# tictacmenthe/F2CNN

Hardware: AMD Instinct MI355X
Metric: audio-seconds/sec through filterbank+envelope (HIP, 1 MI355X per rank); the +CNN figure of BASELINE's metric is value_with_cnn / blocks.cfg4 (higher is better)
Workload: dtype f64 filter state + f64 utterance FFT + f32 row FFT; 1 GPU; cfg3: filterbank + Hilbert envelope + 50 Hz LPF in one call (f32 FFT), batch of 1000 x 1 s utterances per GPU, 128 channels, ENV1 (float64) out; channels=128, lpf_hz=50, launch_batch=1000, outputs_resident_in_hbm=True, parallelism=utterance-sharded x1, no collective, utterances_sent_back_by_the_accuracy_guard=0

## Files before the change

f2cnn_amd/csrc/f2_spectral.hip:

```cpp
#define f2fft f2fft_sp
#undef F2_PLAN13_PASSES
#define F2_PLAN13_PASSES 4
#include <algorithm>
#include <cmath>
#include <complex>
#include <thread>

#include "f2_fft_lds.h"

using namespace f2fft;

namespace {

typedef float f2_f4 __attribute__((ext_vector_type(4)));
constexpr int SPEC_GB = 16;

constexpr int KS_CGROUP = 32;
constexpr int KS_CGROUP_LONG = 8;
constexpr int KS_STORE_AUX = 2;
typedef unsigned int f2_u4 __attribute__((ext_vector_type(4)));
typedef unsigned int f2_u2 __attribute__((ext_vector_type(2)));
__device__ __forceinline__ __amdgpu_buffer_rsrc_t row_buffer(double* y, int n) {
    return __builtin_amdgcn_make_buffer_rsrc(y, 0, n * 8, 0x00020000);
}
__device__ __forceinline__ __amdgpu_buffer_rsrc_t row_buffer_uniform(double* y, int n) {
    const unsigned long long a = (unsigned long long)y;
    const unsigned lo = __builtin_amdgcn_readfirstlane((unsigned)a), hi = __builtin_amdgcn_readfirstlane((unsigned)(a >> 32));
    return row_buffer((double*)(((unsigned long long)hi << 32) | lo), __builtin_amdgcn_readfirstlane(n));
}
__device__ __forceinline__ void store_row_pair_inside(__amdgpu_buffer_rsrc_t r, int i0, double a, double b) {
    const f2_d2 v = {a, b};
    __builtin_amdgcn_raw_buffer_store_b128(__builtin_bit_cast(f2_u4, v), r, i0 * 8, 0, KS_STORE_AUX);
}
__device__ __forceinline__ void store_row_pair_buf(__amdgpu_buffer_rsrc_t r, int n, int i0, double a, double b) {
    if (i0 + 1 < n) {
        const f2_d2 v = {a, b};
        __builtin_amdgcn_raw_buffer_store_b128(__builtin_bit_cast(f2_u4, v), r, i0 * 8, 0, KS_STORE_AUX);
    } else if (i0 < n) {
        __builtin_amdgcn_raw_buffer_store_b64(__builtin_bit_cast(f2_u2, a), r, i0 * 8, 0, KS_STORE_AUX);
    }
}

struct LowpassConsts {
    float qf, b0f;
    float g1, g2, g4, g8;
    double gw, gblk;
};

template <int NT, int NBLK>
constexpr size_t lowpass_tab_lds_bytes() {
    return sizeof(float) * (2 * (size_t)NBLK * (NT / 64) + NBLK);
}

#define F2_DPP_STEP(CTRL)                                                                                                    \
    asm volatile("s_nop 1\n\t"                                                                                               \
                 "v_fmac_f32_dpp %0, %0, %16 " CTRL "\n\t"                                                                   \
                 "v_fmac_f32_dpp %1, %1, %16 " CTRL "\n\t"                                                                   \
                 "v_fmac_f32_dpp %2, %2, %16 " CTRL "\n\t"                                                                   \
                 "v_fmac_f32_dpp %3, %3, %16 " CTRL "\n\t"                                                                   \
                 "v_fmac_f32_dpp %4, %4, %16 " CTRL "\n\t"                                                                   \
                 "v_fmac_f32_dpp %5, %5, %16 " CTRL "\n\t"                                                                   \
                 "v_fmac_f32_dpp %6, %6, %16 " CTRL "\n\t"                                                                   \
                 "v_fmac_f32_dpp %7, %7, %16 " CTRL "\n\t"                                                                   \
                 "v_fmac_f32_dpp %8, %8, %16 " CTRL "\n\t"                                                                   \
                 "v_fmac_f32_dpp %9, %9, %16 " CTRL "\n\t"                                                                   \
                 "v_fmac_f32_dpp %10, %10, %16 " CTRL "\n\t"                                                                 \
                 "v_fmac_f32_dpp %11, %11, %16 " CTRL "\n\t"                                                                 \
                 "v_fmac_f32_dpp %12, %12, %16 " CTRL "\n\t"                                                                 \
                 "v_fmac_f32_dpp %13, %13, %16 " CTRL "\n\t"                                                                 \
                 "v_fmac_f32_dpp %14, %14, %16 " CTRL "\n\t"                                                                 \
                 "v_fmac_f32_dpp %15, %15, %16 " CTRL                                                                        \
                 : "+v"(sc[0]), "+v"(sc[1]), "+v"(sc[2]), "+v"(sc[3]), "+v"(sc[4]), "+v"(sc[5]), "+v"(sc[6]), "+v"(sc[7]),   \
                   "+v"(sc[8]), "+v"(sc[9]), "+v"(sc[10]), "+v"(sc[11]), "+v"(sc[12]), "+v"(sc[13]), "+v"(sc[14]), "+v"(sc[15]) \
                 : "v"(mult))

template <int NT, int NBLK, bool CHAINED = false, bool INSIDE15 = false>
__device__ __forceinline__ float lowpass_pairs_store_tab(const float (&er)[NBLK], const float (&ei)[NBLK], const LowpassConsts& K,
                                                        const f2_f4* __restrict__ lptab, unsigned char* smem,
                                                        double* __restrict__ y, int n, int tid, int ibase = 0,
                                                        double* ychain = nullptr) {
    static_assert(NBLK == 16, "sixteen blocks: one DPP row chains them");
    constexpr int NW = NT / 64;
    float* wtot = reinterpret_cast<float*>(smem);
    float* cwl = wtot + NBLK * NW;
    float* ycar = cwl + NBLK * NW;
    const int lane = tid & 63, wv = tid >> 6;
    const f2_f4 tc = lptab[tid];
    float sc[NBLK];
#pragma unroll
    for (int jj = 0; jj < NBLK; ++jj) sc[jj] = fmaf(K.qf, er[jj], ei[jj]);
    {
        float mult = K.g1;
        F2_DPP_STEP("row_shr:1 row_mask:0xf bank_mask:0xf bound_ctrl:0");
        mult = K.g2;
        F2_DPP_STEP("row_shr:2 row_mask:0xf bank_mask:0xf bound_ctrl:0");
        mult = K.g4;
        F2_DPP_STEP("row_shr:4 row_mask:0xf bank_mask:0xf bound_ctrl:0");
        mult = K.g8;
        F2_DPP_STEP("row_shr:8 row_mask:0xf bank_mask:0xf bound_ctrl:0");
        mult = tc.z;
        F2_DPP_STEP("row_bcast:15 row_mask:0xa bank_mask:0xf");
        mult = tc.w;
        F2_DPP_STEP("row_bcast:31 row_mask:0xc bank_mask:0xf");
    }
    if (lane == 63) {
#pragma unroll
        for (int jj = 0; jj < NBLK; ++jj) wtot[jj * NW + wv] = sc[jj];
    }
    __syncthreads();
    if (tid < NBLK) {
        double c = 0.0;
#pragma unroll
        for (int w2 = 0; w2 < NW; ++w2) {
            cwl[tid * NW + w2] = (float)c;
            c = fma(K.gw, c, (double)wtot[tid * NW + w2]);
        }
        const double G1 = K.gblk, G2 = G1 * G1, G4 = G2 * G2, G8 = G4 * G4;
        double yin = 0.0;
        if constexpr (CHAINED) {
            yin = *ychain;
            if (tid == 0) c = fma(G1, yin, c);
        }
        c = fma(G1, dpp_mov<0x111, 0xF>(c), c);
        c = fma(G2, dpp_mov<0x112, 0xF>(c), c);
        c = fma(G4, dpp_mov<0x114, 0xF>(c), c);
        c = fma(G8, dpp_mov<0x118, 0xF>(c), c);
        const double cprev = dpp_mov<0x111, 0xF>(c);
        if constexpr (CHAINED) {
            ycar[tid] = tid == 0 ? (float)yin : (float)cprev;
            if (tid == NBLK - 1) *ychain = c;
        } else {
            ycar[tid] = (float)cprev;
        }
    }
    __syncthreads();
    const __amdgpu_buffer_rsrc_t yb = CHAINED ? row_buffer_uniform(y, n) : row_buffer(y, n);
    float ymax = 0.f;
#pragma unroll
    for (int jj = 0; jj < NBLK; ++jj) {
        const float cw = cwl[jj * NW + wv];
        const float sin_ = fmaf(tc.x, cw, sc[jj]);
        const float up = dpp_mov<0x138, 0xF>(sin_);
        const float sprev = lane > 0 ? up : cw;
        const float sp = fmaf(tc.y, ycar[jj], sprev);
        const float s0 = fmaf(K.qf, sp, er[jj]);
        const float s1 = fmaf(K.qf, s0, ei[jj]);
        const float y0 = K.b0f * (s0 + sp);
        const float y1 = K.b0f * (s1 + s0);
        const int i0 = ibase + 2 * (tid + NT * jj);
        if constexpr (INSIDE15) {
            if (jj < NBLK - 1) {
                store_row_pair_inside(yb, i0, (double)y0, (double)y1);
                ymax = fmaxf(ymax, fabsf(y1));
            } else {
                store_row_pair_buf(yb, n, i0, (double)y0, (double)y1);
                ymax = fmaxf(ymax, i0 + 1 < n ? fabsf(y1) : (i0 < n ? fabsf(y0) : 0.f));
            }
        } else if constexpr (CHAINED) {
            store_row_pair_buf(yb, n, i0, (double)y0, (double)y1);
            const int lo = ibase + 2 * NT * jj;
            if (lo + 2 * NT <= n) ymax = fmaxf(ymax, fabsf(y1));
            else if (lo < n) ymax = fmaxf(ymax, i0 + 1 < n ? fabsf(y1) : fabsf(y0));
        } else {
            const int lo = ibase + 2 * NT * jj;
            if (lo + 2 * NT <= n) {
                store_row_pair_inside(yb, i0, (double)y0, (double)y1);
                ymax = fmaxf(ymax, fabsf(y1));
            } else if (lo < n) {
                store_row_pair_buf(yb, n, i0, (double)y0, (double)y1);
                ymax = fmaxf(ymax, i0 + 1 < n ? fabsf(y1) : (i0 < n ? fabsf(y0) : 0.f));
            }
        }
    }
    return ymax;
}

struct SpecParams {
    int64_t xpitch;
    int64_t tpitch;
    double* env;
    int* uflag;
    int C;
    int nutt;
    int lpf;
    LowpassConsts lp;
    float tol;
    float* gdump;
    unsigned long long* stamps;
};

__device__ __forceinline__ cpx<float> spectral_bin(cpx<float> X, f2_f4 hu, cpx<float> w, cpx<float> z, const float* __restrict__ rho) {
    const float ur = hu.z, ui = hu.w;
    float tr = fmaf(rho[1], w.re, rho[0]), ti = rho[1] * w.im;
#pragma unroll
    for (int j = 1; j < 4; ++j) {
        const float rr = fmaf(rho[2 * j + 1], w.re, rho[2 * j]), ri = rho[2 * j + 1] * w.im;
        const float nr = fmaf(-ui, ti, fmaf(ur, tr, rr));
        const float ni = fmaf(ui, tr, fmaf(ur, ti, ri));
        tr = nr;
        ti = ni;
    }
    const float qr = ur * tr - ui * ti, qi = ur * ti + ui * tr;
    float yr = hu.x * X.re;
    yr = fmaf(-hu.y, X.im, yr);
    yr = fmaf(z.re, qr, yr);
    yr = fmaf(-z.im, qi, yr);
    float yi = hu.x * X.im;
    yi = fmaf(hu.y, X.re, yi);
    yi = fmaf(z.re, qi, yi);
    yi = fmaf(z.im, qr, yi);
    return {yr, yi};
}

#include "f2_fft13_merged.h"

template <int R0, int J = 0>
__device__ __forceinline__ cpx<float> bin_w(cpx<float> w0, int j) {
    if constexpr (J < R0) {
        if (j == J) return mulw<2 * R0, J>(w0);
        return bin_w<R0, J + 1>(w0, j);
    } else {
        return w0;
    }
}

#define F2_DPP_MAX2(CTRL)                                              \
    asm volatile("s_nop 1\n\t"                                         \
                 "v_max_f32_dpp %0, %0, %0 " CTRL "\n\t"               \
                 "v_max_f32_dpp %1, %1, %1 " CTRL                       \
                 : "+v"(a), "+v"(b))
__device__ __forceinline__ void wave_max63x2(float& a, float& b) {
    F2_DPP_MAX2("row_shr:1 row_mask:0xf bank_mask:0xf bound_ctrl:0");
    F2_DPP_MAX2("row_shr:2 row_mask:0xf bank_mask:0xf bound_ctrl:0");
    F2_DPP_MAX2("row_shr:4 row_mask:0xf bank_mask:0xf bound_ctrl:0");
    F2_DPP_MAX2("row_shr:8 row_mask:0xf bank_mask:0xf bound_ctrl:0");
    F2_DPP_MAX2("row_bcast:15 row_mask:0xa bank_mask:0xf");
    F2_DPP_MAX2("row_bcast:31 row_mask:0xc bank_mask:0xf");
}
__device__ __forceinline__ float wave_max63(float v) {
    asm volatile("s_nop 1\n\t"
                 "v_max_f32_dpp %0, %0, %0 row_shr:1 row_mask:0xf bank_mask:0xf bound_ctrl:0\n\ts_nop 1\n\t"
                 "v_max_f32_dpp %0, %0, %0 row_shr:2 row_mask:0xf bank_mask:0xf bound_ctrl:0\n\ts_nop 1\n\t"
                 "v_max_f32_dpp %0, %0, %0 row_shr:4 row_mask:0xf bank_mask:0xf bound_ctrl:0\n\ts_nop 1\n\t"
                 "v_max_f32_dpp %0, %0, %0 row_shr:8 row_mask:0xf bank_mask:0xf bound_ctrl:0\n\ts_nop 1\n\t"
                 "v_max_f32_dpp %0, %0, %0 row_bcast:15 row_mask:0xa bank_mask:0xf\n\ts_nop 1\n\t"
                 "v_max_f32_dpp %0, %0, %0 row_bcast:31 row_mask:0xc bank_mask:0xf"
                 : "+v"(v));
    return v;
}

template <int R0, int NT, bool PADLAST>
__device__ __forceinline__ float pad_residual(const cpx<float> (&v)[R0], int n, int tid, int odd, float gout) {
    if constexpr (PADLAST) {
        return fmaxf(gout, 2 * (tid + NT * (R0 - 1)) + odd >= n ? fabsf(v[brev<R0>(R0 - 1)].re) : 0.f);
    } else {
        int jmin = (n - 2 * tid - odd + 2 * NT - 1) >> (__builtin_ctz(2 * NT));
        asm volatile("" : "+v"(jmin));
#pragma unroll
        for (int j = R0 / 2; j < R0; ++j) gout = fmaxf(gout, j >= jmin ? fabsf(v[brev<R0>(j)].re) : 0.f);
        return gout;
    }
}

__device__ __forceinline__ void guard_decide(const SpecParams& P, const unsigned* guard, int b, int c) {
    const float gi = __uint_as_float(guard[0]), go = __uint_as_float(guard[1]), gl = __uint_as_float(guard[2]);
    const float den = P.lpf ? gl : gi;
    const bool flag = go > P.tol * den;
    if (flag) P.uflag[b] = 1;
    if (P.gdump) {
        float* g = P.gdump + ((size_t)b * (size_t)P.C + (size_t)c) * 4;
        g[0] = gi;
        g[1] = go;
        g[2] = gl;
        g[3] = flag ? 1.f : 0.f;
    }
}

template <int LOG2H, bool PADLAST>
__global__ __launch_bounds__((threads_for<float, LOG2H>()), (min_waves_for<float, LOG2H>())) void k_spectral_envelope(
    SpecParams P, const cpx<float>* __restrict__ Xall , const f2_f4* __restrict__ HUall,
    const cpx<float>* __restrict__ E , const float* __restrict__ rho_all ,
    const int64_t* __restrict__ offsets, const int* __restrict__ ulist, const f2_f4* __restrict__ lptab,
    const cpx<float>* __restrict__ tw) {
    constexpr int NT = threads_for<float, LOG2H>();
    constexpr int H = 1 << LOG2H;
    constexpr int M = 2 * H;
    constexpr int CS = cpad_size(H);
    constexpr int R0 = 1 << plan_bits(LOG2H, 0);
    constexpr int NB0 = H / R0;
    static_assert(NB0 % NT == 0, "every thread owns whole butterflies of the first pass");
    constexpr int ITER0 = NB0 / NT;
    constexpr int PT = plan_points_per_thread(LOG2H, NT);
    constexpr int NBLK = ITER0 * R0;
    static_assert(PT == NBLK, "register shape");
    constexpr size_t LP = lowpass_tab_lds_bytes<NT, NBLK>();
    constexpr int LDS_BYTES = (int)((size_t)CS * 8 > LP ? (size_t)CS * 8 : LP);
    __shared__ __attribute__((aligned(16))) unsigned char smem[LDS_BYTES];
    constexpr int TWL = plan_tw_lds_count(LOG2H);
    __shared__ __attribute__((aligned(16))) cpx<float> twl[TWL > 0 ? TWL : 1];
    __shared__ unsigned guard[4];
    cpx<float>* lds = reinterpret_cast<cpx<float>*>(smem);

    const int tid = threadIdx.x;
    int u, c;
    {
        constexpr int CG = KS_CGROUP;
        const int nfull = P.C / CG, per = P.nutt * CG;
        const int cg = min((int)(blockIdx.x / per), nfull);
        const int rr = blockIdx.x - cg * per;
        const int gsz = cg < nfull ? CG : P.C - nfull * CG;
        u = rr / gsz;
        c = cg * CG + (rr - u * gsz);
    }
    const int row_id = u * P.C + c;
    const int b = ulist[u];
    const int64_t off = offsets[b];
    const int n = (int)(offsets[b + 1] - off);
    double* __restrict__ y = P.env + ((size_t)P.C * (size_t)off + (size_t)c * (size_t)n);
    const float* __restrict__ rho = rho_all + (size_t)row_id * 8;
    const cpx<float>* __restrict__ Xu = Xall + (size_t)u * P.xpitch;
    const f2_f4* __restrict__ HUc = HUall + (size_t)c * P.tpitch;

    F2_STAMP_ARRAY(st, 8);
    F2_STAMP(st, 0);
    for (int i = tid; i < TWL; i += NT) twl[i] = tw[plan_tw_offset(LOG2H, 1) + i];
    if (tid < 4) guard[tid] = 0u;

    static_assert(ITER0 == 1 && R0 == 16, "one radix-16 butterfly per thread in the first pass");
    constexpr int GB = SPEC_GB, NG = R0 / GB;
    cpx<float> yk[PT], v[PT];
    static_assert(NB0 == NT && plan_npass(LOG2H) >= 3, "fft_pass0_pair + fft_from_pass0");
    cpx<float> vo[PT];
    const unsigned zstep = ((unsigned)NB0 * (unsigned)n) & (M - 1);
    cpx<float> w0 = E[tid];
    cpx<float> z0 = E[__umul24((unsigned)tid, (unsigned)n) & (M - 1)];
    const cpx<float> XH = Xu[H];
    const f2_f4 HUH = HUc[H];
    cpx<float> Xl[2][GB];
    f2_f4 Hl[2][GB];
    unsigned kb = (unsigned)tid;
#pragma unroll
    for (int q = 0; q < GB; ++q) {
        Xl[0][q] = (Xu + q * NB0)[kb];
        Hl[0][q] = (HUc + q * NB0)[kb];
    }
#pragma unroll
    for (int g = 0; g < NG; ++g) {
        if (g + 1 < NG) {
#pragma unroll
            for (int q = 0; q < GB; ++q) {
                Xl[(g + 1) & 1][q] = (Xu + ((g + 1) * GB + q) * NB0)[kb];
                Hl[(g + 1) & 1][q] = (HUc + ((g + 1) * GB + q) * NB0)[kb];
            }
        }
#pragma unroll
        for (int q = 0; q < GB; ++q) {
            const int j = g * GB + q;
            const cpx<float> zj = E[(j * zstep) & (M - 1)];
            const cpx<float> wj = bin_w<R0>(w0, j);
            yk[j] = spectral_bin(Xl[g & 1][q], Hl[g & 1][q], wj, cmul(z0, zj), rho);
            vo[j] = {yk[j].re * wj.re + yk[j].im * wj.im, yk[j].re * wj.im - yk[j].im * wj.re};
#ifdef F2_STAMPS
            if (j == 0 || j == 7) {
                asm volatile("s_nop 0" : "+v"(yk[j].re), "+v"(yk[j].im));
                st[j == 0 ? 1 : 2] = __builtin_amdgcn_s_memrealtime();
                asm volatile("s_nop 0" : "+v"(yk[j].re));
            }
#endif
        }
        asm volatile("" : "+v"(kb), "+v"(w0.re), "+v"(w0.im), "+v"(z0.re), "+v"(z0.im), "+v"(yk[g * GB].re), "+v"(yk[g * GB + GB - 1].re));
    }
#ifdef F2_STAMPS
    asm volatile("s_nop 0" : "+v"(yk[15].re), "+v"(yk[15].im));
    st[3] = __builtin_amdgcn_s_memrealtime();
    asm volatile("s_nop 0" : "+v"(yk[15].re));
#endif
    if (tid == 0) {
        const cpx<float> yh = spectral_bin(XH, HUH, cpx<float>{-1.f, 0.f}, cpx<float>{(n & 1) ? -1.f : 1.f, 0.f}, rho);
        yk[0] = {yk[0].re, yh.re};
    }
    float er[NBLK], ei[NBLK];
    float gin = 0.f, gout = 0.f;
    constexpr bool T0R = derive_tw0<float, LOG2H>();
    {
#pragma unroll
        for (int j = 0; j < R0; ++j) v[j] = {yk[j].re, -yk[j].im};
        if (tid == 0) {
            v[0] = {0.5f * (yk[0].re + yk[0].im), 0.f};
            vo[0] = {0.5f * (yk[0].re - yk[0].im), 0.f};
        }
        F2_STAMP(st, 4);
        int tid_e = tid;
        asm volatile("" : "+v"(tid_e), "+v"(v[0].re), "+v"(vo[PT - 1].im));
        fft_pass0_pair<LOG2H, NT, PT>(tw, tid_e, v, vo);
        fft_from_pass0<LOG2H, PT, NT, T0R>(lds, tw, twl, tid_e, v);
        gout = pad_residual<R0, NT, PADLAST>(v, n, tid, 0, gout);
#pragma unroll
        for (int j = 0; j < R0; ++j) {
            const cpx<float> a = v[brev<R0>(j)];
            er[j] = fsqrt(a.re * a.re + a.im * a.im);
        }
        fft_from_pass0<LOG2H, PT, NT, T0R>(lds, tw, twl, tid_e, vo);
        F2_STAMP(st, 5);
        gout = pad_residual<R0, NT, PADLAST>(vo, n, tid, 1, gout);
#pragma unroll
        for (int j = 0; j < R0; ++j) {
            const cpx<float> a = vo[brev<R0>(j)];
            ei[j] = fsqrt(a.re * a.re + a.im * a.im);
        }
    }
#pragma unroll
    for (int jj = 0; jj < NBLK; ++jj) {
        const int lo = 2 * NT * jj;
        if ((PADLAST && jj < NBLK - 1) || lo + 2 * NT <= n) {
            gin = fmaxf(gin, fmaxf(er[jj], ei[jj]));
        } else if (lo < n) {
            const int i0 = lo + 2 * tid;
            gin = fmaxf(gin, fmaxf(i0 < n ? er[jj] : 0.f, i0 + 1 < n ? ei[jj] : 0.f));
        }
    }
    float glp = 0.f;
    wave_max63x2(gin, gout);
    if ((tid & 63) == 63) {
        __hip_atomic_fetch_max(&guard[0], __float_as_uint(gin), __ATOMIC_RELAXED, __HIP_MEMORY_SCOPE_WORKGROUP);
        __hip_atomic_fetch_max(&guard[1], __float_as_uint(gout), __ATOMIC_RELAXED, __HIP_MEMORY_SCOPE_WORKGROUP);
    }
    F2_STAMP(st, 6);
    if (!P.lpf) {
        const __amdgpu_buffer_rsrc_t yb = row_buffer(y, n);
#pragma unroll
        for (int jj = 0; jj < NBLK; ++jj) {
            if ((PADLAST && jj < NBLK - 1) || 2 * NT * (jj + 1) <= n) store_row_pair_inside(yb, 2 * (tid + NT * jj), (double)er[jj], (double)ei[jj]);
            else if (2 * NT * jj < n) store_row_pair_buf(yb, n, 2 * (tid + NT * jj), (double)er[jj], (double)ei[jj]);
        }
    } else {
        glp = wave_max63(lowpass_pairs_store_tab<NT, NBLK, false, PADLAST>(er, ei, P.lp, lptab, smem, y, n, tid));
    }
    if ((tid & 63) == 63) {
        if (P.lpf) __hip_atomic_fetch_max(&guard[2], __float_as_uint(glp), __ATOMIC_RELAXED, __HIP_MEMORY_SCOPE_WORKGROUP);
        if (__hip_atomic_fetch_add(&guard[3], 1u, __ATOMIC_ACQ_REL, __HIP_MEMORY_SCOPE_WORKGROUP) == (unsigned)(NT / 64 - 1))
            guard_decide(P, guard, b, c);
    }
    F2_STAMP(st, 7);
    F2_STAMP_STORE(st, 8, P.stamps);
}

constexpr int KSL_PARK_AUX = 0;
__device__ __forceinline__ int park_plane(int n, int bank, int r) {
    constexpr int MB = 8192;
    if (bank == 0) return n + r * MB;
    const int nb = n - 4 * MB;
    const int before = r == 0 ? 0 : r == 1 ? (nb + 3) >> 2 : r == 2 ? ((nb + 3) >> 2) + ((nb + 2) >> 2) : nb - (nb >> 2);
    return n + 4 * MB + before;
}
__global__ __launch_bounds__(1024, 4) void k_spectral_envelope_long(
    SpecParams P, const cpx<float>* __restrict__ Xall, const f2_f4* __restrict__ HUall, const cpx<float>* __restrict__ E,
    const float* __restrict__ rho_all, const int64_t* __restrict__ offsets, const int* __restrict__ ulist,
    const f2_f4* __restrict__ lptab, const cpx<float>* __restrict__ tw) {
    constexpr int LOG2Q = 14, NT = 1024, Q = 1 << LOG2Q, H = 2 * Q, M = 2 * H;
    static_assert(threads_for<float, LOG2Q>() == NT, "the 16-16-4-16 plan on 1024 threads");
    constexpr int CS = cpad_size(Q);
    constexpr int R0 = 16, NB0 = Q / R0, PT = 16, NBLK = 16;
    static_assert(NB0 == NT && plan_points_per_thread(LOG2Q, NT) == PT, "one radix-16 butterfly per thread in the first pass");
    constexpr size_t LP = lowpass_tab_lds_bytes<NT, NBLK>();
    constexpr int LDS_BYTES = (int)((size_t)CS * 8 > LP ? (size_t)CS * 8 : LP);
    __shared__ __attribute__((aligned(16))) unsigned char smem[LDS_BYTES];
    constexpr int TWL = plan_tw_lds_count(LOG2Q);
    __shared__ __attribute__((aligned(16))) cpx<float> twl[TWL];
    __shared__ unsigned guard[4];
    __shared__ double ychain;
    cpx<float>* lds = reinterpret_cast<cpx<float>*>(smem);

    const int tid = threadIdx.x;
    int u, c;
    {
        constexpr int CG = KS_CGROUP_LONG;
        const int nfull = P.C / CG, per = P.nutt * CG;
        const int cg = min((int)(blockIdx.x / per), nfull);
        const int rr = blockIdx.x - cg * per;
        const int gsz = cg < nfull ? CG : P.C - nfull * CG;
        u = rr / gsz;
        c = cg * CG + (rr - u * gsz);
    }
    const int row_id = u * P.C + c;
    const int b = ulist[u];
    const int64_t off = offsets[b];
    const int n = (int)(offsets[b + 1] - off);
    double* __restrict__ y = P.env + ((size_t)P.C * (size_t)off + (size_t)c * (size_t)n);
    const float* __restrict__ rho = rho_all + (size_t)row_id * 8;
    const cpx<float>* __restrict__ Xu = Xall + (size_t)u * P.xpitch;
    const f2_f4* __restrict__ HUc = HUall + (size_t)c * P.tpitch;

    for (int i = tid; i < TWL; i += NT) twl[i] = tw[plan_tw_offset(LOG2Q, 1) + i];
    if (tid < 4) guard[tid] = 0u;
    if (tid == 0) ychain = 0.0;

    const unsigned zstep = ((unsigned)NB0 * (unsigned)n) & (M - 1);
    cpx<float> w0 = E[tid];
    cpx<float> z0 = E[((unsigned)tid * (unsigned)n) & (M - 1)];
    const cpx<float> zq = E[((unsigned)Q * (unsigned)n) & (M - 1)];
    float yh = 0.f;
    if (tid == 0) yh = spectral_bin(Xu[H], HUc[H], cpx<float>{-1.f, 0.f}, cpx<float>{(n & 1) ? -1.f : 1.f, 0.f}, rho).re;
    constexpr bool T0R = derive_tw0<float, LOG2Q>();
    float gin = 0.f, gout = 0.f;
    unsigned kb = (unsigned)tid;
    F2_STAMP_ARRAY(st, 8);
    F2_STAMP(st, 0);
#pragma unroll 1
    for (int p = 0; p < 2; ++p) {
        cpx<float> v[PT], vo[PT];
        constexpr int GB = 4;
#pragma unroll
        for (int g = 0; g < R0 / GB; ++g) {
            cpx<float> Xl[2][GB];
            f2_f4 Hl[2][GB];
#pragma unroll
            for (int q = 0; q < GB; ++q) {
                Xl[0][q] = (Xu + (g * GB + q) * NB0)[kb];
                Hl[0][q] = (HUc + (g * GB + q) * NB0)[kb];
// ... 7 lines not shown
                const cpx<float> z = cmul(z0, E[(j * zstep) & (M - 1)]);
                const cpx<float> ya = spectral_bin(Xl[0][q], Hl[0][q], w, z, rho);
                const cpx<float> yb2 = spectral_bin(Xl[1][q], Hl[1][q], cpx<float>{w.im, -w.re}, cmul(z, zq), rho);
                cpx<float> cp = {ya.re, -ya.im};
                if (j == 0 && tid == 0) cp = {0.5f * (ya.re + (p ? -yh : yh)), 0.f};
                const cpx<float> cr = p ? cpx<float>{-yb2.im, -yb2.re} : cpx<float>{yb2.re, -yb2.im};
                const cpx<float> sm = cp + cr, df = cp - cr;
                const cpx<float> w2 = cmul(w, w);
                v[j] = p ? cmul(sm, w) : sm;
                vo[j] = cmul(df, p ? cmul(w2, w) : w2);
            }
            asm volatile("" : "+v"(kb), "+v"(w0.re), "+v"(w0.im), "+v"(z0.re), "+v"(z0.im), "+v"(v[g * GB].re), "+v"(vo[g * GB + GB - 1].im));
        }
        int tid_e = tid;
        asm volatile("" : "+v"(tid_e), "+v"(v[0].re), "+v"(vo[PT - 1].im));
        if (p == 0) F2_STAMP(st, 1);
        else F2_STAMP(st, 3);
        fft_pass0_pair<LOG2Q, NT, PT>(tw, tid_e, v, vo);
#pragma unroll
        for (int half = 0; half < 2; ++half) {
            if (half == 0) fft_from_pass0<LOG2Q, PT, NT, T0R>(lds, tw, twl, tid_e, v);
            else fft_from_pass0<LOG2Q, PT, NT, T0R>(lds, tw, twl, tid_e, vo);
            const int r = p + 2 * half;
            const __amdgpu_buffer_rsrc_t yb = row_buffer_uniform(y, n);
            const int pv0 = 4 * (park_plane(n, 0, r) + tid), pv1 = 4 * (park_plane(n, 1, r) + tid);
#pragma unroll
            for (int j = 0; j < R0; ++j) {
                const cpx<float> a = half ? vo[brev<R0>(j)] : v[brev<R0>(j)];
                const float e = fsqrt(a.re * a.re + a.im * a.im);
                const bool in = 4 * (tid + NT * j) + r < n;
                __builtin_amdgcn_raw_buffer_store_b32(__float_as_uint(e), yb, in ? (j < 8 ? pv0 : pv1) : 0x7ffffff0, 4 * NT * (j & 7),
                                                      KSL_PARK_AUX);
                gin = fmaxf(gin, in ? e : 0.f);
                if (j >= 8 && 4 * NT * (j + 1) > n) gout = fmaxf(gout, in ? 0.f : fabsf(a.re));
            }
        }
        if (p == 0) F2_STAMP(st, 2);
        else F2_STAMP(st, 4);
    }
    gin = wave_max63(gin);
    gout = wave_max63(gout);
    if ((tid & 63) == 63) {
        atomicMax(&guard[0], __float_as_uint(gin));
        atomicMax(&guard[1], __float_as_uint(gout));
    }
    __builtin_amdgcn_fence(__ATOMIC_RELEASE, "workgroup");
    __syncthreads();
    __builtin_amdgcn_fence(__ATOMIC_ACQUIRE, "workgroup");
    float glp = 0.f;
#pragma unroll 1
    for (int sw = 0; sw < 2; ++sw) {
        const int ibase = sw * 2 * NT * NBLK;
        const __amdgpu_buffer_rsrc_t yb = row_buffer_uniform(y, n);
        float er[NBLK], ei[NBLK];
        const int rl = 2 * (tid & 1);
        const int pva = 4 * (park_plane(n, sw, rl) + (tid >> 1)), pvb = 4 * (park_plane(n, sw, rl + 1) + (tid >> 1));
#pragma unroll
        for (int jj = 0; jj < NBLK; ++jj) {
            const int i0 = ibase + 2 * (tid + NT * jj);
            er[jj] = __uint_as_float(__builtin_amdgcn_raw_buffer_load_b32(yb, i0 < n ? pva : 0x7ffffff0, 2 * NT * jj, KSL_PARK_AUX));
            ei[jj] = __uint_as_float(__builtin_amdgcn_raw_buffer_load_b32(yb, i0 + 1 < n ? pvb : 0x7ffffff0, 2 * NT * jj, KSL_PARK_AUX));
        }
        if (!P.lpf) {
            __syncthreads();
#pragma unroll
            for (int jj = 0; jj < NBLK; ++jj) store_row_pair_buf(yb, n, ibase + 2 * (tid + NT * jj), (double)er[jj], (double)ei[jj]);
        } else {
            glp = fmaxf(glp, lowpass_pairs_store_tab<NT, NBLK, true>(er, ei, P.lp, lptab, smem, y, n, tid, ibase, &ychain));
        }
        __syncthreads();
        if (sw == 0) F2_STAMP(st, 5);
        else F2_STAMP(st, 6);
    }
    if (P.lpf) glp = wave_max63(glp);
    if ((tid & 63) == 63) {
        if (P.lpf) __hip_atomic_fetch_max(&guard[2], __float_as_uint(glp), __ATOMIC_RELAXED, __HIP_MEMORY_SCOPE_WORKGROUP);
        if (__hip_atomic_fetch_add(&guard[3], 1u, __ATOMIC_ACQ_REL, __HIP_MEMORY_SCOPE_WORKGROUP) == (unsigned)(NT / 64 - 1))
            guard_decide(P, guard, b, c);
    }
    F2_STAMP(st, 7);
    F2_STAMP_STORE(st, 8, P.stamps);
}

template <typename WaveT, int LOG2HS, int LOGD>
__global__ __launch_bounds__((threads_for<double, LOG2HS>())) void k_utterance_spectrum(const WaveT* __restrict__ wave,
                                                                                      const int64_t* __restrict__ offsets,
                                                                                      const int* __restrict__ ulist,
                                                                                      cpx<float>* __restrict__ X, int64_t xpitch,
                                                                                      cpx<double>* __restrict__ Xpart,
                                                                                      const cpx<double>* __restrict__ tw) {
    constexpr int LOG2H = LOG2HS;
    constexpr int D = 1 << LOGD;
    constexpr int NT = threads_for<double, LOG2H>();
    constexpr int H = 1 << LOG2H;
    constexpr int CS = cpad_size(H);
    constexpr int R0 = 1 << plan_bits(LOG2H, 0);
    constexpr int NB0 = H / R0;
    constexpr int ITER0 = (NB0 + NT - 1) / NT;
    constexpr int PT = plan_points_per_thread(LOG2H, NT);
    constexpr bool FULL0 = NB0 % NT == 0;
    __shared__ __attribute__((aligned(16))) cpx<double> lds[CS];
    constexpr int TWL = plan_tw_lds_count(LOG2H);
    __shared__ __attribute__((aligned(16))) cpx<double> twl[TWL > 0 ? TWL : 1];
    const cpx<double>* __restrict__ V = tw + plan_tw_total(LOG2H);
    const int tid = threadIdx.x;
    const int ul = blockIdx.x >> LOGD, ph = blockIdx.x & (D - 1);
    const int b = ulist[ul];
    const int64_t off = offsets[b];
    const int n = (int)(offsets[b + 1] - off);
    const WaveT* __restrict__ x = wave + off;
    for (int i = tid; i < TWL; i += NT) twl[i] = tw[plan_tw_offset(LOG2H, 1) + i];
    cpx<double> v[PT];
#pragma unroll
    for (int i = 0; i < ITER0; ++i) {
        const int bf = tid + i * NT;
        if (FULL0 || bf < NB0) {
#pragma unroll
            for (int j = 0; j < R0; ++j) {
                const int i0 = D * 2 * (bf + j * NB0) + ph, i1 = i0 + D;
                v[i * R0 + j] = {i0 < n ? (double)x[i0] : 0.0, i1 < n ? (double)x[i1] : 0.0};
            }
        }
    }
    fft_all<double, LOG2H, false, PT, NT, false>(lds, tw, twl, tid, v);
    cpx<float>* __restrict__ Xo = X + (size_t)ul * xpitch;
    cpx<double>* __restrict__ Xp = Xpart + (size_t)blockIdx.x * (H + 1);
    for (int k = 1 + tid; k <= H / 2; k += NT) {
        const cpx<double> zk = lds[cpad(k)], zh = lds[cpad(H - k)];
        const cpx<double> e = {0.5 * (zk.re + zh.re), 0.5 * (zk.im - zh.im)};
        const cpx<double> o = {0.5 * (zk.im + zh.im), -0.5 * (zk.re - zh.re)};
        const cpx<double> w = V[k];
        const cpx<double> wo = {o.re * w.re - o.im * w.im, o.re * w.im + o.im * w.re};
        if constexpr (LOGD == 0) {
            Xo[k] = {(float)(e.re + wo.re), (float)(e.im + wo.im)};
            Xo[H - k] = {(float)(e.re - wo.re), (float)(-(e.im - wo.im))};
        } else {
            Xp[k] = {e.re + wo.re, e.im + wo.im};
            Xp[H - k] = {e.re - wo.re, -(e.im - wo.im)};
        }
    }
    if (tid == 0) {
        const cpx<double> z0 = lds[cpad(0)];
        if constexpr (LOGD == 0) {
            Xo[0] = {(float)(z0.re + z0.im), 0.f};
            Xo[H] = {(float)(z0.re - z0.im), 0.f};
        } else {
            Xp[0] = {z0.re + z0.im, 0.0};
            Xp[H] = {z0.re - z0.im, 0.0};
        }
    }
}

template <int LOG2HS, int LOGD>
__global__ __launch_bounds__(256) void k_spectrum_combine(const cpx<double>* __restrict__ Xpart, const cpx<double>* __restrict__ e64,
                                                          cpx<float>* __restrict__ X, int64_t xpitch) {
    constexpr int D = 1 << LOGD, HS = 1 << LOG2HS, H = D * HS, M = 2 * H;
    const int ul = blockIdx.y;
    const int k = blockIdx.x * 256 + threadIdx.x;
    if (k > H) return;
    const int kk = k & (2 * HS - 1);
    double re = 0.0, im = 0.0;
#pragma unroll
    for (int ph = 0; ph < D; ++ph) {
        const cpx<double>* __restrict__ Xp = Xpart + ((size_t)ul * D + ph) * (HS + 1);
        cpx<double> xp = kk <= HS ? Xp[kk] : Xp[2 * HS - kk];
        if (kk > HS) xp.im = -xp.im;
        const cpx<double> w = e64[(ph * k) & (M - 1)];
        re += xp.re * w.re - xp.im * w.im;
        im += xp.re * w.im + xp.im * w.re;
    }
    X[(size_t)ul * xpitch + k] = {(float)re, (float)im};
}

constexpr int TAIL_TB = 32;
constexpr int TAIL_WAVES = 4;

template <typename WaveT>
__global__ __launch_bounds__((64 * TAIL_WAVES)) void k_tail_state(const WaveT* __restrict__ wave, const int64_t* __restrict__ offsets,
                                                                const double* __restrict__ coefs, int C, int groups,
                                                                const int* __restrict__ ulist, int nutt,
                                                                const int* __restrict__ Lgroup, float* __restrict__ rho,
                                                                double two_over_m) {
    __shared__ double xss[TAIL_WAVES][TAIL_TB];
    const int lane = threadIdx.x & 63;
    const int wid = __builtin_amdgcn_readfirstlane(threadIdx.x >> 6);
    const int unit = blockIdx.x * TAIL_WAVES + wid;
    if (unit >= nutt * groups) return;
    const int ul = unit / groups, g = unit - ul * groups;
    const int b = ulist[ul];
    const int64_t off = offsets[b];
    const int64_t N = offsets[b + 1] - off;
    const int cc = g * 64 + lane;
    const int c = min(cc, C - 1);
    const double* k = coefs + (size_t)c * 10;
    const double rB0 = 1.0 / k[6];
    const double b0 = k[0] * rB0, a1 = k[7] * rB0, a2 = k[8] * rB0;
    const double c1 = k[1] / k[0], c2 = k[2] / k[0], c3 = k[3] / k[0], c4 = k[4] / k[0];
    const double scale = (b0 * b0) * (b0 * b0) / k[9] * two_over_m;
    double* xs = xss[wid];
    const WaveT* w = wave + off;
    const int64_t L = min((int64_t)Lgroup[g], N);
    const int64_t nblk = (L + TAIL_TB - 1) / TAIL_TB;
    const int64_t t_begin = N - nblk * TAIL_TB;
// ... 186 lines not shown
    return true;
}

static int spectral_tables(f2_ctx* ctx, const double* d_coefs, int C, int log2h, f2_spec_tables** out) {
    for (auto& t : ctx->spec_tabs)
        if (t.log2h == log2h && t.C == C && t.coefs == ctx->coefs_host) {
            *out = &t;
            return F2_OK;
        }
    if (ctx->spec_tabs.size() >= 6) {
        F2_HIP(ctx, hipStreamSynchronize(ctx->stream));
        ctx->spec_tabs.erase(ctx->spec_tabs.begin());
    }
    f2_spec_tables t;
    t.log2h = log2h;
    t.C = C;
    t.coefs = ctx->coefs_host;
    std::vector<int> Lg;
    if (!f2_spectral_supports_coefs(t.coefs, C, &Lg, nullptr)) return f2_fail(ctx, F2_ERR_INVALID, "coefficient table not eligible");
    const int H = 1 << log2h, M = 2 * H;
    t.tpitch = H + 8;
    F2_TRY(f2_reserve(ctx, t.hu, sizeof(float) * 4 * (size_t)C * (size_t)t.tpitch));
    F2_TRY(f2_reserve(ctx, t.e, sizeof(float) * 2 * (size_t)M));
    F2_TRY(f2_reserve(ctx, t.lgroup, sizeof(int) * Lg.size()));
    if (log2h > 13) F2_TRY(f2_reserve(ctx, t.e64, sizeof(double) * 2 * (size_t)M));
    hipLaunchKernelGGL(k_spectral_tables, dim3((unsigned)((M + 255) / 256), (unsigned)(C + 1)), dim3(256), 0, ctx->stream, d_coefs, C, H,
                       t.tpitch, (f2_f4*)t.hu.ptr, (cpx<float>*)t.e.ptr, (cpx<double>*)t.e64.ptr);
    F2_HIP(ctx, hipGetLastError());
    F2_TRY(f2_upload_async(ctx, t.lgroup.ptr, Lg.data(), sizeof(int) * Lg.size()));
    ctx->spec_tabs.push_back(std::move(t));
    *out = &ctx->spec_tabs.back();
    return F2_OK;
}

static int lowpass_table(f2_ctx* ctx, double a1, double b0, int nt, int sp, LowpassConsts* K, const f2_f4** d_tab) {
    const long double q = -(long double)a1;
    K->qf = (float)q;
    K->b0f = (float)b0;
    K->g1 = (float)powl(q, sp);
    K->g2 = (float)powl(q, 2 * sp);
    K->g4 = (float)powl(q, 4 * sp);
    K->g8 = (float)powl(q, 8 * sp);
    K->gw = (double)powl(q, 64 * sp);
    K->gblk = (double)powl(q, sp * nt);
    f2_scratch& slot = ctx->spec_lptab;
    double& slot_a1 = ctx->spec_lptab_a1;
    *d_tab = (const f2_f4*)slot.ptr;
    constexpr int TMAX = 1024;
    if (slot.ptr && slot_a1 == a1) return F2_OK;
    std::vector<float> tab((size_t)TMAX * 4);
    for (int t = 0; t < TMAX; ++t) {
        const int lane = t & 63;
        tab[4 * (size_t)t] = (float)powl(q, sp * (lane + 1));
        tab[4 * (size_t)t + 1] = (float)powl(q, sp * t);
        tab[4 * (size_t)t + 2] = (float)powl(q, sp * ((lane & 15) + 1));
        tab[4 * (size_t)t + 3] = (float)powl(q, sp * ((lane & 31) + 1));
    }
    F2_TRY(f2_reserve(ctx, slot, sizeof(float) * tab.size()));
    F2_TRY(f2_upload_async(ctx, slot.ptr, tab.data(), sizeof(float) * tab.size()));
    slot_a1 = a1;
    *d_tab = (const f2_f4*)slot.ptr;
    return F2_OK;
}

template <typename WaveT, int LOG2H>
static int launch_group(f2_ctx* ctx, const WaveT* d_wave, const int64_t* d_offsets, const double* d_coefs, int C,
                        const int* d_ulist, int nutt, int64_t min_n, int lpf, double b0, double a1, double* d_env, int* d_uflag,
                        float tol, cpx<float>* d_X, float* d_rho) {
    constexpr int H = 1 << LOG2H, M = 2 * H;
    f2_spec_tables* tab = nullptr;
    F2_TRY(spectral_tables(ctx, d_coefs, C, LOG2H, &tab));
    constexpr int LOGD = LOG2H > 13 ? LOG2H - 13 : 0, LOG2HS = LOG2H - LOGD;
    constexpr int FFTLOG = LOG2H == 15 ? 14 : LOG2H;
    F2_TRY(ensure_twiddles<double>(ctx, LOG2HS, ctx->tw_sp[1][LOG2HS]));
    F2_TRY(ensure_twiddles<float>(ctx, FFTLOG, ctx->tw_sp[0][FFTLOG]));
    const int64_t xpitch = H + 8;
    const int groups = (C + 63) / 64;
    F2_TRY(f2_prof_begin(ctx, F2_K_SPECTRUM));
    cpx<double>* d_part = nullptr;
    if constexpr (LOGD > 0) {
        F2_TRY(f2_reserve(ctx, ctx->spec_xpart, sizeof(double) * 2 * ((size_t)(1 << LOG2HS) + 1) * (size_t)nutt << LOGD));
        d_part = (cpx<double>*)ctx->spec_xpart.ptr;
    }
    hipLaunchKernelGGL((k_utterance_spectrum<WaveT, LOG2HS, LOGD>), dim3((unsigned)nutt << LOGD), dim3(threads_for<double, LOG2HS>()),
                       0, ctx->stream, d_wave, d_offsets, d_ulist, d_X, xpitch, d_part,
                       (const cpx<double>*)ctx->tw_sp[1][LOG2HS].ptr);
    F2_HIP(ctx, hipGetLastError());
    if constexpr (LOGD > 0) {
        hipLaunchKernelGGL((k_spectrum_combine<LOG2HS, LOGD>), dim3((unsigned)((H + 256) / 256), (unsigned)nutt), dim3(256), 0,
                           ctx->stream, (const cpx<double>*)d_part, (const cpx<double>*)tab->e64.ptr, d_X, xpitch);
        F2_HIP(ctx, hipGetLastError());
    }
    F2_TRY(f2_prof_end(ctx, F2_K_SPECTRUM));
    F2_TRY(f2_prof_begin(ctx, F2_K_TAIL));
    const int units = nutt * groups;
    hipLaunchKernelGGL((k_tail_state<WaveT>), dim3((unsigned)((units + TAIL_WAVES - 1) / TAIL_WAVES)), dim3(64 * TAIL_WAVES), 0,
                       ctx->stream, d_wave, d_offsets, d_coefs, C, groups, d_ulist, nutt, (const int*)tab->lgroup.ptr, d_rho,
                       2.0 / M);
    F2_HIP(ctx, hipGetLastError());
    F2_TRY(f2_prof_end(ctx, F2_K_TAIL));
    SpecParams P;
    P.xpitch = xpitch;
    P.tpitch = tab->tpitch;
    P.env = d_env;
    P.uflag = d_uflag;
    P.C = C;
    P.nutt = nutt;
    P.lpf = lpf;
    const f2_f4* d_lptab = nullptr;
    F2_TRY(lowpass_table(ctx, a1, b0, threads_for<float, FFTLOG>(), 2, &P.lp, &d_lptab));
    P.tol = tol;
    P.gdump = ctx->opt_spectral_guard_dump ? (float*)ctx->spec_gdump.ptr : nullptr;
    P.stamps = nullptr;
#ifdef F2_STAMPS
    F2_TRY(f2_stamps_buffer(ctx, (size_t)nutt * C, 8, &P.stamps));
#endif
    F2_TRY(f2_prof_begin(ctx, F2_K_FUSED));
    if constexpr (LOG2H == 15)
        hipLaunchKernelGGL(k_spectral_envelope_long, dim3((unsigned)((size_t)nutt * C)), dim3(threads_for<float, FFTLOG>()), 0,
                           ctx->stream, P, (const cpx<float>*)d_X, (const f2_f4*)tab->hu.ptr, (const cpx<float>*)tab->e.ptr,
                           (const float*)d_rho, d_offsets, d_ulist, d_lptab, (const cpx<float>*)ctx->tw_sp[0][FFTLOG].ptr);
    else if (min_n >= 15 * (M / 16))
        hipLaunchKernelGGL((k_spectral_envelope<FFTLOG, true>), dim3((unsigned)((size_t)nutt * C)), dim3(threads_for<float, FFTLOG>()), 0,
                           ctx->stream, P, (const cpx<float>*)d_X, (const f2_f4*)tab->hu.ptr, (const cpx<float>*)tab->e.ptr,
                           (const float*)d_rho, d_offsets, d_ulist, d_lptab, (const cpx<float>*)ctx->tw_sp[0][FFTLOG].ptr);
    else
        hipLaunchKernelGGL((k_spectral_envelope<FFTLOG, false>), dim3((unsigned)((size_t)nutt * C)), dim3(threads_for<float, FFTLOG>()), 0,
                           ctx->stream, P, (const cpx<float>*)d_X, (const f2_f4*)tab->hu.ptr, (const cpx<float>*)tab->e.ptr,
                           (const float*)d_rho, d_offsets, d_ulist, d_lptab, (const cpx<float>*)ctx->tw_sp[0][FFTLOG].ptr);
    F2_HIP(ctx, hipGetLastError());
    F2_TRY(f2_prof_end(ctx, F2_K_FUSED));
#ifdef F2_STAMPS
    static const char* names_s[8] = {"", "bin 0 ready", "bin 7 ready", "bin 15 ready", "transform inputs", "both transforms + even magnitudes", "odd magnitudes + guard", "lpf+stores"};
    static const char* names_l[8] = {"", "spectrum r=0,2", "transforms r=0,2 + parking", "spectrum r=1,3", "transforms r=1,3 + parking", "low-pass sweep 0", "low-pass sweep 1", "flag"};
    F2_TRY(f2_stamps_report(ctx, P.stamps, (size_t)nutt * C, 8, LOG2H == 15 ? names_l : names_s, "[stamps KS]",
                            "mean ticks (10 ns) per workgroup:", true));
#endif
    return F2_OK;
}

int f2_launch_spectral(f2_ctx* ctx, const void* d_wave, int wave_dtype, const int64_t* d_offsets, const double* d_coefs,
                       int C, const int* d_ulist, int nutt, int64_t min_n, int log2h, int lpf, double cutoff_hz, double* d_env,
                       int* d_uflag) {
    if (nutt <= 0) return F2_OK;
    const double k = lpf ? tan(3.14159265358979323846 * cutoff_hz / 16000.0) : 0.0;
    const double b0 = k / (1.0 + k), a1 = (k - 1.0) / (k + 1.0);
    const float tol = ctx->opt_spectral_tol;
    const int H = 1 << log2h;
    F2_TRY(f2_reserve(ctx, ctx->spec_x, sizeof(float) * 2 * (size_t)(H + 8) * (size_t)nutt));
    F2_TRY(f2_reserve(ctx, ctx->spec_rho, sizeof(float) * 8 * (size_t)nutt * (size_t)C));
    cpx<float>* d_X = (cpx<float>*)ctx->spec_x.ptr;
    float* d_rho = (float*)ctx->spec_rho.ptr;
#define F2_SPEC_CASE(L)                                                                                                          \
    case L:                                                                                                                      \
        return wave_dtype == F2_WAVE_I16                                                                                         \
                   ? launch_group<int16_t, L>(ctx, (const int16_t*)d_wave, d_offsets, d_coefs, C, d_ulist, nutt, min_n, lpf, b0, \
                                              a1, d_env, d_uflag, tol, d_X, d_rho)                                              \
                   : launch_group<double, L>(ctx, (const double*)d_wave, d_offsets, d_coefs, C, d_ulist, nutt, min_n, lpf, b0,   \
                                             a1, d_env, d_uflag, tol, d_X, d_rho);
    switch (log2h) {
        F2_SPEC_CASE(12)
        F2_SPEC_CASE(13)
        F2_SPEC_CASE(14)
        F2_SPEC_CASE(15)
        default:
            return f2_fail(ctx, F2_ERR_UNSUPPORTED, "spectral path: length class 2^%d not built", log2h + 1);
    }
// ... 3 lines not shown
```

Baseline: 205,200 audio-seconds/s.

## Front-pad utterances in the spectral path to drop per-bin phase rotation

Places each utterance at the end of the FFT frame, zero-padding at the front instead of the back, so the ringing term's output-position phase factor becomes unity. This removes the per-bin E-table lookup and complex multiply (z0, zj) from the spectral-bin loop, and replaces the tail-boundary masking with front-boundary masking for stores, guard maxima and padding residuals. The store loop in the lowpass is rotated so the partial first block is handled last. It changes indexing across the spectrum kernel and the envelope kernel, and it risks boundary mistakes at the front edge.

```diff
diff --git a/f2cnn_amd/csrc/f2_spectral.hip b/f2cnn_amd/csrc/f2_spectral.hip
--- a/f2cnn_amd/csrc/f2_spectral.hip
+++ b/f2cnn_amd/csrc/f2_spectral.hip
@@ -38,6 +38,14 @@
         __builtin_amdgcn_raw_buffer_store_b128(__builtin_bit_cast(f2_u4, v), r, i0 * 8, 0, KS_STORE_AUX);
     } else if (i0 < n) {
         __builtin_amdgcn_raw_buffer_store_b64(__builtin_bit_cast(f2_u2, a), r, i0 * 8, 0, KS_STORE_AUX);
+    }
+}
+__device__ __forceinline__ void store_row_pair_front(__amdgpu_buffer_rsrc_t r, int t0, double a, double b) {
+    if (t0 >= 0) {
+        const f2_d2 v = {a, b};
+        __builtin_amdgcn_raw_buffer_store_b128(__builtin_bit_cast(f2_u4, v), r, t0 * 8, 0, KS_STORE_AUX);
+    } else if (t0 == -1) {
+        __builtin_amdgcn_raw_buffer_store_b64(__builtin_bit_cast(f2_u2, b), r, 0, 0, KS_STORE_AUX);
     }
 }
 
@@ -74,11 +82,11 @@
                    "+v"(sc[8]), "+v"(sc[9]), "+v"(sc[10]), "+v"(sc[11]), "+v"(sc[12]), "+v"(sc[13]), "+v"(sc[14]), "+v"(sc[15]) \
                  : "v"(mult))
 
-template <int NT, int NBLK, bool CHAINED = false, bool INSIDE15 = false>
+template <int NT, int NBLK, bool CHAINED = false, bool INSIDE_BUT_FIRST = false>
 __device__ __forceinline__ float lowpass_pairs_store_tab(const float (&er)[NBLK], const float (&ei)[NBLK], const LowpassConsts& K,
                                                         const f2_f4* __restrict__ lptab, unsigned char* smem,
                                                         double* __restrict__ y, int n, int tid, int ibase = 0,
-                                                        double* ychain = nullptr) {
+                                                        double* ychain = nullptr, int np = 0) {
     static_assert(NBLK == 16, "sixteen blocks: one DPP row chains them");
     constexpr int NW = NT / 64;
     float* wtot = reinterpret_cast<float*>(smem);
@@ -137,7 +145,8 @@
     const __amdgpu_buffer_rsrc_t yb = CHAINED ? row_buffer_uniform(y, n) : row_buffer(y, n);
     float ymax = 0.f;
 #pragma unroll
-    for (int jj = 0; jj < NBLK; ++jj) {
+    for (int k = 0; k < NBLK; ++k) {
+        const int jj = INSIDE_BUT_FIRST ? (k + 1) % NBLK : k;
         const float cw = cwl[jj * NW + wv];
         const float sin_ = fmaf(tc.x, cw, sc[jj]);
         const float up = dpp_mov<0x138, 0xF>(sin_);
@@ -148,28 +157,16 @@
         const float y0 = K.b0f * (s0 + sp);
         const float y1 = K.b0f * (s1 + s0);
         const int i0 = ibase + 2 * (tid + NT * jj);
-        if constexpr (INSIDE15) {
-            if (jj < NBLK - 1) {
-                store_row_pair_inside(yb, i0, (double)y0, (double)y1);
-                ymax = fmaxf(ymax, fabsf(y1));
-            } else {
-                store_row_pair_buf(yb, n, i0, (double)y0, (double)y1);
-                ymax = fmaxf(ymax, i0 + 1 < n ? fabsf(y1) : (i0 < n ? fabsf(y0) : 0.f));
-            }
-        } else if constexpr (CHAINED) {
+        if constexpr (CHAINED) {
             store_row_pair_buf(yb, n, i0, (double)y0, (double)y1);
             const int lo = ibase + 2 * NT * jj;
             if (lo + 2 * NT <= n) ymax = fmaxf(ymax, fabsf(y1));
             else if (lo < n) ymax = fmaxf(ymax, i0 + 1 < n ? fabsf(y1) : fabsf(y0));
         } else {
-            const int lo = ibase + 2 * NT * jj;
-            if (lo + 2 * NT <= n) {
-                store_row_pair_inside(yb, i0, (double)y0, (double)y1);
-                ymax = fmaxf(ymax, fabsf(y1));
-            } else if (lo < n) {
-                store_row_pair_buf(yb, n, i0, (double)y0, (double)y1);
-                ymax = fmaxf(ymax, i0 + 1 < n ? fabsf(y1) : (i0 < n ? fabsf(y0) : 0.f));
-            }
+            ymax = fmaxf(ymax, fabsf(y1));
+            const int lo = 2 * NT * jj;
+            if ((INSIDE_BUT_FIRST && jj > 0) || jj >= NBLK / 2 || lo >= np) store_row_pair_inside(yb, i0 - np, (double)y0, (double)y1);
+            else if (lo + 2 * NT > np) store_row_pair_front(yb, i0 - np, (double)y0, (double)y1);
         }
     }
     return ymax;
@@ -189,7 +186,7 @@
     unsigned long long* stamps;
 };
 
-__device__ __forceinline__ cpx<float> spectral_bin(cpx<float> X, f2_f4 hu, cpx<float> w, cpx<float> z, const float* __restrict__ rho) {
+__device__ __forceinline__ cpx<float> ringing_bin(f2_f4 hu, cpx<float> w, const float* __restrict__ rho) {
     const float ur = hu.z, ui = hu.w;
     float tr = fmaf(rho[1], w.re, rho[0]), ti = rho[1] * w.im;
 #pragma unroll
@@ -200,7 +197,17 @@
         tr = nr;
         ti = ni;
     }
-    const float qr = ur * tr - ui * ti, qi = ur * ti + ui * tr;
+    return {ur * tr - ui * ti, ur * ti + ui * tr};
+}
+__device__ __forceinline__ cpx<float> spectral_bin(cpx<float> X, f2_f4 hu, cpx<float> w, const float* __restrict__ rho) {
+    const cpx<float> q = ringing_bin(hu, w, rho);
+    const float yr = fmaf(-hu.y, X.im, fmaf(hu.x, X.re, q.re));
+    const float yi = fmaf(hu.y, X.re, fmaf(hu.x, X.im, q.im));
+    return {yr, yi};
+}
+__device__ __forceinline__ cpx<float> spectral_bin(cpx<float> X, f2_f4 hu, cpx<float> w, cpx<float> z, const float* __restrict__ rho) {
+    const cpx<float> q = ringing_bin(hu, w, rho);
+    const float qr = q.re, qi = q.im;
     float yr = hu.x * X.re;
     yr = fmaf(-hu.y, X.im, yr);
     yr = fmaf(z.re, qr, yr);
@@ -249,16 +256,27 @@
     return v;
 }
 
-template <int R0, int NT, bool PADLAST>
-__device__ __forceinline__ float pad_residual(const cpx<float> (&v)[R0], int n, int tid, int odd, float gout) {
-    if constexpr (PADLAST) {
-        return fmaxf(gout, 2 * (tid + NT * (R0 - 1)) + odd >= n ? fabsf(v[brev<R0>(R0 - 1)].re) : 0.f);
+template <int R0, int NT, bool PADFIRST>
+__device__ __forceinline__ float pad_residual(const cpx<float> (&v)[R0], int np, int tid, int odd, float gout) {
+    if constexpr (PADFIRST) {
+        return fmaxf(gout, 2 * tid + odd < np ? fabsf(v[brev<R0>(0)].re) : 0.f);
     } else {
-        int jmin = (n - 2 * tid - odd + 2 * NT - 1) >> (__builtin_ctz(2 * NT));
-        asm volatile("" : "+v"(jmin));
-#pragma unroll
-        for (int j = R0 / 2; j < R0; ++j) gout = fmaxf(gout, j >= jmin ? fabsf(v[brev<R0>(j)].re) : 0.f);
+        int jlim = (np - 2 * tid - odd + 2 * NT - 1) >> (__builtin_ctz(2 * NT));
+        asm volatile("" : "+v"(jlim));
+#pragma unroll
+        for (int j = 0; j < R0 / 2; ++j) gout = fmaxf(gout, j < jlim ? fabsf(v[brev<R0>(j)].re) : 0.f);
         return gout;
+    }
+}
+
+template <int NT, int NBLK, bool FIRSTONLY>
+__device__ __forceinline__ void zero_front_padding(float (&er)[NBLK], float (&ei)[NBLK], int np, int tid) {
+    int d = 2 * tid - np;
+    asm volatile("" : "+v"(d));
+#pragma unroll
+    for (int jj = 0; jj < (FIRSTONLY ? 1 : NBLK / 2); ++jj) {
+        er[jj] = d >= -2 * NT * jj ? er[jj] : 0.f;
+        ei[jj] = d >= -2 * NT * jj - 1 ? ei[jj] : 0.f;
     }
 }
 
@@ -276,7 +294,7 @@
     }
 }
 
-template <int LOG2H, bool PADLAST>
+template <int LOG2H, bool PADFIRST>
 __global__ __launch_bounds__((threads_for<float, LOG2H>()), (min_waves_for<float, LOG2H>())) void k_spectral_envelope(
     SpecParams P, const cpx<float>* __restrict__ Xall , const f2_f4* __restrict__ HUall,
     const cpx<float>* __restrict__ E , const float* __restrict__ rho_all ,
@@ -316,6 +334,7 @@
     const int b = ulist[u];
     const int64_t off = offsets[b];
     const int n = (int)(offsets[b + 1] - off);
+    const int np = M - n;
     double* __restrict__ y = P.env + ((size_t)P.C * (size_t)off + (size_t)c * (size_t)n);
     const float* __restrict__ rho = rho_all + (size_t)row_id * 8;
     const cpx<float>* __restrict__ Xu = Xall + (size_t)u * P.xpitch;
@@ -331,9 +350,7 @@
     cpx<float> yk[PT], v[PT];
     static_assert(NB0 == NT && plan_npass(LOG2H) >= 3, "fft_pass0_pair + fft_from_pass0");
     cpx<float> vo[PT];
-    const unsigned zstep = ((unsigned)NB0 * (unsigned)n) & (M - 1);
     cpx<float> w0 = E[tid];
-    cpx<float> z0 = E[__umul24((unsigned)tid, (unsigned)n) & (M - 1)];
     const cpx<float> XH = Xu[H];
     const f2_f4 HUH = HUc[H];
     cpx<float> Xl[2][GB];
@@ -356,9 +373,8 @@
 #pragma unroll
         for (int q = 0; q < GB; ++q) {
             const int j = g * GB + q;
-            const cpx<float> zj = E[(j * zstep) & (M - 1)];
             const cpx<float> wj = bin_w<R0>(w0, j);
-            yk[j] = spectral_bin(Xl[g & 1][q], Hl[g & 1][q], wj, cmul(z0, zj), rho);
+            yk[j] = spectral_bin(Xl[g & 1][q], Hl[g & 1][q], wj, rho);
             vo[j] = {yk[j].re * wj.re + yk[j].im * wj.im, yk[j].re * wj.im - yk[j].im * wj.re};
 #ifdef F2_STAMPS
             if (j == 0 || j == 7) {
@@ -368,7 +384,7 @@
             }
 #endif
         }
-        asm volatile("" : "+v"(kb), "+v"(w0.re), "+v"(w0.im), "+v"(z0.re), "+v"(z0.im), "+v"(yk[g * GB].re), "+v"(yk[g * GB + GB - 1].re));
+        asm volatile("" : "+v"(kb), "+v"(w0.re), "+v"(w0.im), "+v"(yk[g * GB].re), "+v"(yk[g * GB + GB - 1].re));
     }
 #ifdef F2_STAMPS
     asm volatile("s_nop 0" : "+v"(yk[15].re), "+v"(yk[15].im));
@@ -376,7 +392,7 @@
     asm volatile("s_nop 0" : "+v"(yk[15].re));
 #endif
     if (tid == 0) {
-        const cpx<float> yh = spectral_bin(XH, HUH, cpx<float>{-1.f, 0.f}, cpx<float>{(n & 1) ? -1.f : 1.f, 0.f}, rho);
+        const cpx<float> yh = spectral_bin(XH, HUH, cpx<float>{-1.f, 0.f}, rho);
         yk[0] = {yk[0].re, yh.re};
     }
     float er[NBLK], ei[NBLK];
@@ -394,7 +410,7 @@
         asm volatile("" : "+v"(tid_e), "+v"(v[0].re), "+v"(vo[PT - 1].im));
         fft_pass0_pair<LOG2H, NT, PT>(tw, tid_e, v, vo);
         fft_from_pass0<LOG2H, PT, NT, T0R>(lds, tw, twl, tid_e, v);
-        gout = pad_residual<R0, NT, PADLAST>(v, n, tid, 0, gout);
+        gout = pad_residual<R0, NT, PADFIRST>(v, np, tid, 0, gout);
 #pragma unroll
         for (int j = 0; j < R0; ++j) {
             const cpx<float> a = v[brev<R0>(j)];
@@ -402,23 +418,16 @@
         }
         fft_from_pass0<LOG2H, PT, NT, T0R>(lds, tw, twl, tid_e, vo);
         F2_STAMP(st, 5);
-        gout = pad_residual<R0, NT, PADLAST>(vo, n, tid, 1, gout);
+        gout = pad_residual<R0, NT, PADFIRST>(vo, np, tid, 1, gout);
 #pragma unroll
         for (int j = 0; j < R0; ++j) {
             const cpx<float> a = vo[brev<R0>(j)];
             ei[j] = fsqrt(a.re * a.re + a.im * a.im);
         }
     }
-#pragma unroll
-    for (int jj = 0; jj < NBLK; ++jj) {
-        const int lo = 2 * NT * jj;
-        if ((PADLAST && jj < NBLK - 1) || lo + 2 * NT <= n) {
-            gin = fmaxf(gin, fmaxf(er[jj], ei[jj]));
-        } else if (lo < n) {
-            const int i0 = lo + 2 * tid;
-            gin = fmaxf(gin, fmaxf(i0 < n ? er[jj] : 0.f, i0 + 1 < n ? ei[jj] : 0.f));
-        }
-    }
+    zero_front_padding<NT, NBLK, PADFIRST>(er, ei, np, tid);
+#pragma unroll
+    for (int jj = 0; jj < NBLK; ++jj) gin = fmaxf(gin, fmaxf(er[jj], ei[jj]));
     float glp = 0.f;
     wave_max63x2(gin, gout);
     if ((tid & 63) == 63) {
@@ -430,11 +439,12 @@
         const __amdgpu_buffer_rsrc_t yb = row_buffer(y, n);
 #pragma unroll
         for (int jj = 0; jj < NBLK; ++jj) {
-            if ((PADLAST && jj < NBLK - 1) || 2 * NT * (jj + 1) <= n) store_row_pair_inside(yb, 2 * (tid + NT * jj), (double)er[jj], (double)ei[jj]);
-            else if (2 * NT * jj < n) store_row_pair_buf(yb, n, 2 * (tid + NT * jj), (double)er[jj], (double)ei[jj]);
+            const int t0 = 2 * (tid + NT * jj) - np;
+            if ((PADFIRST && jj > 0) || jj >= NBLK / 2 || 2 * NT * jj >= np) store_row_pair_inside(yb, t0, (double)er[jj], (double)ei[jj]);
+            else if (2 * NT * (jj + 1) > np) store_row_pair_front(yb, t0, (double)er[jj], (double)ei[jj]);
         }
     } else {
-        glp = wave_max63(lowpass_pairs_store_tab<NT, NBLK, false, PADLAST>(er, ei, P.lp, lptab, smem, y, n, tid));
+        glp = wave_max63(lowpass_pairs_store_tab<NT, NBLK, false, PADFIRST>(er, ei, P.lp, lptab, smem, y, n, tid, 0, nullptr, np));
     }
     if ((tid & 63) == 63) {
         if (P.lpf) __hip_atomic_fetch_max(&guard[2], __float_as_uint(glp), __ATOMIC_RELAXED, __HIP_MEMORY_SCOPE_WORKGROUP);
@@ -608,7 +618,7 @@
     F2_STAMP_STORE(st, 8, P.stamps);
 }
 
-template <typename WaveT, int LOG2HS, int LOGD>
+template <typename WaveT, int LOG2HS, int LOGD, bool FRONT>
 __global__ __launch_bounds__((threads_for<double, LOG2HS>())) void k_utterance_spectrum(const WaveT* __restrict__ wave,
                                                                                       const int64_t* __restrict__ offsets,
                                                                                       const int* __restrict__ ulist,
@@ -635,6 +645,7 @@
     const int64_t off = offsets[b];
     const int n = (int)(offsets[b + 1] - off);
     const WaveT* __restrict__ x = wave + off;
+    const int np = FRONT ? 2 * D * H - n : 0;
     for (int i = tid; i < TWL; i += NT) twl[i] = tw[plan_tw_offset(LOG2H, 1) + i];
     cpx<double> v[PT];
 #pragma unroll
@@ -643,8 +654,8 @@
         if (FULL0 || bf < NB0) {
 #pragma unroll
             for (int j = 0; j < R0; ++j) {
-                const int i0 = D * 2 * (bf + j * NB0) + ph, i1 = i0 + D;
-                v[i * R0 + j] = {i0 < n ? (double)x[i0] : 0.0, i1 < n ? (double)x[i1] : 0.0};
+                const int i0 = D * 2 * (bf + j * NB0) + ph - np, i1 = i0 + D;
+                v[i * R0 + j] = {i0 >= 0 && i0 < n ? (double)x[i0] : 0.0, i1 >= 0 && i1 < n ? (double)x[i1] : 0.0};
             }
         }
     }
@@ -997,7 +1008,8 @@
         F2_TRY(f2_reserve(ctx, ctx->spec_xpart, sizeof(double) * 2 * ((size_t)(1 << LOG2HS) + 1) * (size_t)nutt << LOGD));
         d_part = (cpx<double>*)ctx->spec_xpart.ptr;
     }
-    hipLaunchKernelGGL((k_utterance_spectrum<WaveT, LOG2HS, LOGD>), dim3((unsigned)nutt << LOGD), dim3(threads_for<double, LOG2HS>()),
+    constexpr bool FRONT = LOG2H != 15;
+    hipLaunchKernelGGL((k_utterance_spectrum<WaveT, LOG2HS, LOGD, FRONT>), dim3((unsigned)nutt << LOGD), dim3(threads_for<double, LOG2HS>()),
                        0, ctx->stream, d_wave, d_offsets, d_ulist, d_X, xpitch, d_part,
                        (const cpx<double>*)ctx->tw_sp[1][LOG2HS].ptr);
     F2_HIP(ctx, hipGetLastError());
```

New measurement: 214,700 audio-seconds/s (median of 6 runs). 1.05x the previous value.
